# NeRdTheNed/deft4j

Measured on NVIDIA B200. Metric: input MB/s optimised (-m NONE), higher is better.
Workload: dtype u8

## Files before the change

### deft4j_b200/csrc/deft4cu.cu

```cuda
#include <algorithm>
#include <cstdio>
#include <cstdlib>
#include <cstring>
#include <memory>
#include <chrono>
#include <mutex>
#include <string>
#include <thread>
#include <vector>

#include "../../include/deft4cu.h"

namespace d4 {
static thread_local std::string g_err;
static void set_error(const std::string& s) { g_err = s; }
}

#include "write.cuh"
#include "checksum.cuh"

namespace d4 {

static int g_device = -1;
static int g_sms = 148;
// ... 255 lines not shown
    std::vector<uint32_t> chain_off;
    uint32_t parse_rewalks = 0, parse_walkers = 0;

    int parse() {
        HostTimer ht("parse");
        release_model();
        too_big = false;
        cudaEvent_t ev[4];
        for (auto& e : ev) cudaEventCreate(&e);
        descs.assign(n + 1, StreamDesc{});
        infos.assign(n, StreamInfo{});
        D4_CUDA_CHECK(dalloc(&d_gerr, 8, cs));
        D4_CUDA_CHECK(cudaMemsetAsync(d_gerr, 0, 8 * sizeof(int), cs));
        uint64_t seg_bytes = 128 << 10;
        if (const char* e = getenv("D4_SEG_BYTES")) seg_bytes = std::max<uint64_t>(64, strtoull(e, nullptr, 10));
        const uint64_t seg_bits = seg_bytes * 8;
        const uint64_t spec_max_bits = 4 * seg_bits + (1 << 20);
        wdescs.clear();
        std::vector<uint32_t> w0(n), spec_list, all_list;
        for (uint32_t i = 0; i < n; i++) {
            const uint32_t nseg = in_len[i] <= seg_bytes ? 1u : (uint32_t)((in_len[i] + seg_bytes - 1) / seg_bytes);
            w0[i] = (uint32_t)wdescs.size();
            for (uint32_t j = 0; j < nseg; j++) {
                StreamDesc d{};
                d.in_off = in_off[i]; d.in_len = in_len[i];
                d.start_bit = j == 0 ? 0 : BIT_NONE;
                d.stop_bit = nseg == 1 ? BIT_NONE : (uint64_t)(j + 1) * seg_bits;
                d.walker0 = w0[i]; d.nseg = nseg; d.spec = j == 0 ? 0 : 1;
                if (nseg == 1) { d.blk_cap = in_len[i] / 4096 + 8; d.chunk_cap = in_len[i] * 8 / CHUNK_BITS + d.blk_cap + 8; }
                else { d.blk_cap = seg_bytes / 2048 + 8; d.chunk_cap = 4 * seg_bits / CHUNK_BITS + d.blk_cap + 8; }
                if (j) spec_list.push_back((uint32_t)wdescs.size());
                all_list.push_back((uint32_t)wdescs.size());
                wdescs.push_back(d);
            }
        }
        const uint32_t W = (uint32_t)wdescs.size();
        parse_walkers = W; parse_rewalks = 0;
        std::vector<uint32_t> wstream(W);
        for (uint32_t i = 0; i < n; i++) for (uint32_t j = 0; j < wdescs[w0[i]].nseg; j++) wstream[w0[i] + j] = i;
        winfos.assign(W, StreamInfo{});
        uint32_t* d_list = nullptr;
        D4_CUDA_CHECK(dalloc(&d_descs, (size_t)W, cs));
        D4_CUDA_CHECK(dalloc(&d_infos, (size_t)W, cs));
        D4_CUDA_CHECK(dalloc(&d_list, (size_t)W, cs));
        cudaEventRecord(ev[0], cs);
        if (!spec_list.empty()) {
            D4_CUDA_CHECK(cudaMemcpyAsync(d_descs, wdescs.data(), sizeof(StreamDesc) * W, cudaMemcpyHostToDevice, cs));
            D4_CUDA_CHECK(cudaMemcpyAsync(d_list, spec_list.data(), 4 * spec_list.size(), cudaMemcpyHostToDevice, cs));
            LAUNCH(k_find, (unsigned)spec_list.size(), FIND_NT, cs, d_in, d_descs, d_list, seg_bits);
            std::vector<StreamDesc> tmp(W);
            D4_CUDA_CHECK(cudaMemcpyAsync(tmp.data(), d_descs, sizeof(StreamDesc) * W, cudaMemcpyDeviceToHost, cs));
            D4_CUDA_CHECK(cudaStreamSynchronize(cs));
            for (uint32_t w : spec_list) wdescs[w].start_bit = tmp[w].start_bit;
        }
        chain.clear(); chain_off.assign(n + 1, 0);
        std::vector<std::vector<uint32_t>> chains(n);
        std::vector<uint8_t> trunc(n, 0);
        for (int attempt = 0;; attempt++) {
            uint64_t bt = 0, ct = 0;
            for (uint32_t w = 0; w < W; w++) {
                wdescs[w].blk_base = bt; bt += wdescs[w].blk_cap;
                wdescs[w].chunk_base = ct; ct += wdescs[w].chunk_cap;
            }
            dfree(d_blocks, cs); dfree(d_chunks, cs);
            D4_CUDA_CHECK(dalloc(&d_blocks, bt, cs));
            D4_CUDA_CHECK(dalloc(&d_chunks, ct, cs));
            D4_CUDA_CHECK(cudaMemcpyAsync(d_descs, wdescs.data(), sizeof(StreamDesc) * W, cudaMemcpyHostToDevice, cs));
            D4_CUDA_CHECK(cudaMemcpyAsync(d_list, all_list.data(), 4 * (size_t)W, cudaMemcpyHostToDevice, cs));
            if (W) LAUNCH_SM(k_count, W, PARSE_NT, WIN_BYTES + WIN_SLACK + 16, cs, d_in, d_descs, d_infos, d_blocks, d_chunks, d_list, seg_bits, spec_max_bits);
            D4_CUDA_CHECK(cudaMemcpyAsync(winfos.data(), d_infos, sizeof(StreamInfo) * W, cudaMemcpyDeviceToHost, cs));
            D4_CUDA_CHECK(cudaStreamSynchronize(cs));
            if (stage && cs == own_cs) { host_release(stage); stage = nullptr; }
            std::vector<uint32_t> cur(n), pending;
            std::vector<uint8_t> fin(n, 0);
            for (uint32_t i = 0; i < n; i++) { chains[i].assign(1, w0[i]); cur[i] = w0[i]; }
            bool overflow = false;
            while (true) {
                pending.clear();
                for (uint32_t i = 0; i < n; i++) {
                    if (fin[i]) continue;
                    while (true) {
                        const StreamInfo& wi = winfos[cur[i]];
                        const StreamDesc& wd = wdescs[cur[i]];
                        if (wi.n_blocks > wd.blk_cap || wi.n_chunks > wd.chunk_cap) { overflow = true; fin[i] = 1; break; }
                        if (wi.status != ST_OK || wi.final_seen) { fin[i] = 1; break; }
                        if (wi.end_bit + 3 > in_len[i] * 8) { fin[i] = 2; break; }
                        uint64_t j = wi.end_bit / seg_bits;
                        if (j >= wd.nseg) j = wd.nseg - 1;
                        const uint32_t nx = w0[i] + (uint32_t)j;
                        if (nx <= cur[i]) {
                            set_error("parse chain did not advance");
                            return DEFT4CU_ERR_CUDA;
                        }
                        chains[i].push_back(nx);
                        cur[i] = nx;
                        if (wdescs[nx].start_bit == wi.end_bit && winfos[nx].status != ST_NONE && winfos[nx].status != ST_ABORT)
                            continue;
                        wdescs[nx].start_bit = wi.end_bit;
                        wdescs[nx].spec = 0;
                        pending.push_back(nx);
                        break;
                    }
                }
                if (pending.empty()) break;
                parse_rewalks += (uint32_t)pending.size();
                for (uint32_t w : pending)
                    D4_CUDA_CHECK(cudaMemcpyAsync(d_descs + w, &wdescs[w], sizeof(StreamDesc), cudaMemcpyHostToDevice, cs));
                D4_CUDA_CHECK(cudaMemcpyAsync(d_list, pending.data(), 4 * pending.size(), cudaMemcpyHostToDevice, cs));
                LAUNCH_SM(k_count, (unsigned)pending.size(), PARSE_NT, WIN_BYTES + WIN_SLACK + 16, cs, d_in, d_descs, d_infos, d_blocks, d_chunks, d_list, seg_bits, spec_max_bits);
                for (uint32_t w : pending)
                    D4_CUDA_CHECK(cudaMemcpyAsync(&winfos[w], d_infos + w, sizeof(StreamInfo), cudaMemcpyDeviceToHost, cs));
                D4_CUDA_CHECK(cudaStreamSynchronize(cs));
            }
            for (uint32_t i = 0; i < n; i++) trunc[i] = fin[i] == 2;
            if (!overflow) break;
            if (attempt == 3) { set_error("block/chunk capacity retry failed"); return DEFT4CU_ERR_CUDA; }
            for (uint32_t w = 0; w < W; w++) {
                if (winfos[w].status == ST_NONE) continue;
                wdescs[w].blk_cap = std::max<uint64_t>(wdescs[w].blk_cap, winfos[w].n_blocks + 8);
                wdescs[w].chunk_cap = std::max<uint64_t>(wdescs[w].chunk_cap, 2 * winfos[w].n_chunks + 8);
            }
        }
        for (uint32_t i = 0; i < n; i++) {
            StreamInfo& si = infos[i];
            si = StreamInfo{};
            si.status = ST_OK;
            for (uint32_t w : chains[i]) {
                const StreamInfo& wi = winfos[w];
                si.n_blocks += wi.n_blocks; si.n_syms += wi.n_syms; si.out_len += wi.out_len; si.n_chunks += wi.n_chunks;
                si.end_bit = wi.end_bit;
                if (wi.status != ST_OK) { si.status = wi.status >= ST_NONE ? ST_PARSE : wi.status; break; }
            }
            if (trunc[i] && si.status == ST_OK) si.status = ST_PARSE;
            if (si.out_len > 0xF0000000ull && si.status == ST_OK) si.status = ST_UNSUPPORTED;
            si.total_bits = si.end_bit;
            si.consumed = (si.end_bit + 7) >> 3;
            chain_off[i] = (uint32_t)chain.size();
            if (si.status == ST_OK) chain.insert(chain.end(), chains[i].begin(), chains[i].end());
        }
        chain_off[n] = (uint32_t)chain.size();
        dfree(d_list, cs);
        cudaEventRecord(ev[1], cs);
        uint64_t sb = 0, ob = 0;
        for (uint32_t i = 0; i < n; i++) {
            descs[i].sym_base = sb; descs[i].out_base = ob;
            for (uint32_t c = chain_off[i]; c < chain_off[i + 1]; c++) {
                StreamDesc& wd = wdescs[chain[c]];
                wd.sym_base = sb; wd.out_base = ob; wd.stream_out_base = descs[i].out_base;
                sb += winfos[chain[c]].n_syms; ob += winfos[chain[c]].out_len;
            }
        }
        descs[n].sym_base = sb; descs[n].out_base = ob;
        nsym_total = sb; nout_total = ob;
        uint64_t ob_max = 0xF8000000ull;
        if (const char* e = getenv("D4_MAX_DECODED")) ob_max = std::min<uint64_t>(ob_max, strtoull(e, nullptr, 10));
        if (ob >= ob_max) {
            too_big = true;
            for (uint32_t i = 0; i < n; i++) if (infos[i].status == ST_OK) infos[i].status = ST_UNSUPPORTED;
            set_error("decoded size of the batch exceeds 4 GiB; split the batch");
            return DEFT4CU_ERR_UNSUPPORTED;
        }
        D4_CUDA_CHECK(cudaMemcpyAsync(d_descs, wdescs.data(), sizeof(StreamDesc) * W, cudaMemcpyHostToDevice, cs));
        D4_CUDA_CHECK(dalloc(&d_sym, sb, cs));
        D4_CUDA_CHECK(dalloc(&d_symout, sb, cs));
        D4_CUDA_CHECK(dalloc(&d_out, ob + 16, cs));
        std::vector<EmitJob> jobs;
        blk_stream.clear();
// ... 316 lines not shown
    }
};

}

using namespace d4;

struct deft4cu_stream {
    std::shared_ptr<Batch> batch;
    uint32_t idx;
    bool written = false;
};
struct deft4cu_device_batch {
    std::shared_ptr<Batch> batch;
};

extern "C" {

int deft4cu_init(int device) {
    std::lock_guard<std::mutex> lk(g_mu);
    int count = 0;
    cudaError_t e = cudaGetDeviceCount(&count);
    if (e != cudaSuccess || count == 0) {
        set_error(std::string("no CUDA device: ") + cudaGetErrorString(e));
        return DEFT4CU_ERR_CUDA;
    }
    if (device < 0 || device >= count) { set_error("bad device index"); return DEFT4CU_ERR_ARG; }
    D4_CUDA_CHECK(cudaSetDevice(device));
    cudaDeviceProp p;
    D4_CUDA_CHECK(cudaGetDeviceProperties(&p, device));
    g_sms = p.multiProcessorCount;
    D4_CUDA_CHECK(cudaFuncSetAttribute(k_count, cudaFuncAttributeMaxDynamicSharedMemorySize, WIN_BYTES + WIN_SLACK + 16));
    cudaMemPool_t pool;
    if (cudaDeviceGetDefaultMemPool(&pool, device) == cudaSuccess) {
        uint64_t thr = ~0ull;
        cudaMemPoolSetAttribute(pool, cudaMemPoolAttrReleaseThreshold, &thr);
    }
    if (getenv("D4_DEBUG_LIMITS")) {
        size_t st = 0, hp = 0;
        cudaDeviceGetLimit(&st, cudaLimitStackSize);
        cudaDeviceGetLimit(&hp, cudaLimitMallocHeapSize);
        cudaFuncAttributes fa;
        cudaFuncGetAttributes(&fa, k_opt_blocks);
        fprintf(stderr, "[deft4cu] stack limit %zu heap %zu; k_opt_blocks local %zu regs %d smem %zu\n", st, hp, fa.localSizeBytes, fa.numRegs, fa.sharedSizeBytes);
        if (getenv("D4_STACK")) { cudaDeviceSetLimit(cudaLimitStackSize, atoi(getenv("D4_STACK"))); }
    }
    g_device = device;
    return DEFT4CU_OK;
}
const char* deft4cu_last_error(void) { return g_err.c_str(); }
const char* deft4cu_version(void) { return "deft4cu 0.2 (sm_100a)"; }

int deft4cu_debug_trace_begin(uint32_t cap) {
    int rc = ensure_init();
    if (rc) return rc;
    if (g_trace_dev) { cudaFree(g_trace_dev); g_trace_dev = nullptr; }
    D4_CUDA_CHECK(cudaMalloc((void**)&g_trace_dev, 16ull * cap));
    g_trace_dev_cap = cap;
    unsigned zero = 0;
    D4_CUDA_CHECK(cudaMemcpyToSymbol(g_trace, &g_trace_dev, sizeof(g_trace_dev)));
    D4_CUDA_CHECK(cudaMemcpyToSymbol(g_trace_cap, &cap, sizeof(cap)));
    D4_CUDA_CHECK(cudaMemcpyToSymbol(g_trace_n, &zero, sizeof(zero)));
    return DEFT4CU_OK;
}
int deft4cu_debug_trace_end(int64_t* dst, uint32_t cap, uint32_t* n) {
    if (!g_trace_dev) { set_error("trace not armed"); return DEFT4CU_ERR_ARG; }
    D4_CUDA_CHECK(cudaDeviceSynchronize());
    unsigned cnt = 0;
    D4_CUDA_CHECK(cudaMemcpyFromSymbol(&cnt, g_trace_n, sizeof(cnt)));
    long long* null = nullptr;
    D4_CUDA_CHECK(cudaMemcpyToSymbol(g_trace, &null, sizeof(null)));
    if (n) *n = cnt;
    uint32_t m = std::min(std::min(cnt, cap), g_trace_dev_cap);
    if (m) D4_CUDA_CHECK(cudaMemcpy(dst, g_trace_dev, 16ull * m, cudaMemcpyDeviceToHost));
    cudaFree(g_trace_dev);
    g_trace_dev = nullptr;
    return DEFT4CU_OK;
}

uint64_t deft4cu_debug_engine_launches(void) { return g_opt_launches; }

int deft4cu_debug_prof(uint64_t* dst, uint32_t n, int reset) {
#ifdef D4_PROF
    unsigned long long h[64];
    D4_CUDA_CHECK(cudaDeviceSynchronize());
    D4_CUDA_CHECK(cudaMemcpyFromSymbol(h, g_prof, sizeof(h)));
    for (uint32_t i = 0; i < n && i < 64; i++) dst[i] = h[i];
    if (reset) { memset(h, 0, sizeof h); D4_CUDA_CHECK(cudaMemcpyToSymbol(g_prof, h, sizeof(h))); }
    return DEFT4CU_OK;
#else
    (void)dst; (void)n; (void)reset;
    set_error("not a -DD4_PROF build");
    return DEFT4CU_ERR_ARG;
#endif
}

int deft4cu_stream_parse_batch(const uint8_t* const* data, const uint64_t* len, uint32_t n, deft4cu_stream** handles,
                               int32_t* status, uint64_t* consumed) {
    int rc = ensure_init();
    if (rc) return rc;
    auto b = std::make_shared<Batch>();
    rc = b->upload(data, len, n);
    if (rc) return rc;
    rc = b->parse();
    if (rc && rc != DEFT4CU_ERR_UNSUPPORTED) return rc;
    for (uint32_t i = 0; i < n; i++) {
        int st = b->infos[i].status;
        if (status) status[i] = st;
        if (consumed) consumed[i] = b->infos[i].consumed;
        handles[i] = nullptr;
        if (st == ST_OK) handles[i] = new deft4cu_stream{b, i};
    }
    return DEFT4CU_OK;
}
int deft4cu_stream_parse(const uint8_t* data, uint64_t len, deft4cu_stream** out, uint64_t* consumed) {
    int32_t st = 0;
    uint64_t c = 0;
    *out = nullptr;
    int rc = deft4cu_stream_parse_batch(&data, &len, 1, out, &st, &c);
    if (consumed) *consumed = c;
    if (rc) return rc;
    return st;
}
void deft4cu_stream_free(deft4cu_stream* s) { delete s; }

int deft4cu_stream_optimise_batch(deft4cu_stream* const* s, uint32_t n, uint32_t flags, int64_t* saved_bits) {
    std::vector<Batch*> batches;
    for (uint32_t i = 0; i < n; i++) {
        if (!s[i]) return DEFT4CU_ERR_ARG;
        if (std::find(batches.begin(), batches.end(), s[i]->batch.get()) == batches.end()) batches.push_back(s[i]->batch.get());
    }
    if (batches.size() > 1) {
        bool fresh = true;
        for (Batch* b : batches) fresh = fresh && !b->optimised && b->parsed;
        for (uint32_t i = 0; i < n && fresh; i++)
            for (uint32_t k = 0; k < i; k++) if (s[k] == s[i]) fresh = false;
        if (fresh) {
            std::vector<std::pair<Batch*, uint32_t>> src(n);
            for (uint32_t i = 0; i < n; i++) src[i] = {s[i]->batch.get(), s[i]->idx};
            auto nb = std::make_shared<Batch>();
            int rc = nb->upload_from(src);
            if (rc == DEFT4CU_OK) rc = nb->parse();
            bool same = rc == DEFT4CU_OK;
            for (uint32_t i = 0; i < n && same; i++) same = nb->infos[i].status == ST_OK;
            if (same) {
                for (uint32_t i = 0; i < n; i++) { s[i]->batch = nb; s[i]->idx = i; }
                batches.assign(1, nb.get());
            } else if (rc != DEFT4CU_OK && rc != DEFT4CU_ERR_UNSUPPORTED) return rc;
        }
    }
    int worst = DEFT4CU_OK;
    for (Batch* b : batches) {
        std::vector<uint8_t> sel(b->n, 0);
        for (uint32_t i = 0; i < n; i++) if (s[i]->batch.get() == b) sel[s[i]->idx] = 1;
        int rc = b->optimise(flags, sel);
        if (rc) worst = rc;
    }
    for (uint32_t i = 0; i < n; i++) {
        s[i]->written = false;
        if (saved_bits) saved_bits[i] = s[i]->batch->sstate[s[i]->idx].saved_bits;
    }
    return worst;
}
int deft4cu_stream_optimise(deft4cu_stream* s, uint32_t flags, int64_t* saved_bits) {
    return deft4cu_stream_optimise_batch(&s, 1, flags, saved_bits);
}
int64_t deft4cu_stream_size_bits(const deft4cu_stream* s) { return (int64_t)s->batch->sstate[s->idx].total_bits; }
uint64_t deft4cu_stream_uncompressed_len(const deft4cu_stream* s) { return s->batch->infos[s->idx].out_len; }
int deft4cu_stream_uncompressed(const deft4cu_stream* s, uint8_t* dst, uint64_t cap) {
    Batch& b = *s->batch;
    uint64_t len = b.infos[s->idx].out_len;
// ... 249 lines not shown
```

### deft4j_b200/csrc/parse.cuh

```cuda
#pragma once
#include "common.cuh"

namespace d4 {

constexpr int PARSE_NT = 1024;
constexpr int CHUNK_BITS = 256;

struct DecTab {
    uint32_t first[16];
    uint16_t count[16];
    uint16_t offs[16];
    uint16_t symtab[MAX_LL];
};

__device__ inline void build_dectab(const uint8_t* lens, int n, DecTab& t) {
    for (int l = 0; l < 16; l++) { t.count[l] = 0; t.first[l] = 0; t.offs[l] = 0; }
    for (int i = 0; i < n; i++) if (lens[i] > 0 && lens[i] < 16) t.count[lens[i]]++;
    uint32_t next = 0;
    int lastShift = 0, off = 0;
    for (int l = 1; l < 16; l++) {
        t.offs[l] = (uint16_t)off;
        off += t.count[l];
        if (t.count[l] == 0) continue;
        next <<= (l - lastShift);
        lastShift = l;
        t.first[l] = next;
        next += t.count[l];
    }
    uint16_t fill[16];
    for (int l = 0; l < 16; l++) fill[l] = t.offs[l];
    for (int i = 0; i < n; i++) if (lens[i] > 0 && lens[i] < 16) t.symtab[fill[lens[i]]++] = (uint16_t)i;
}

__device__ __forceinline__ int decode_sym(const DecTab& t, uint64_t w, int* len) {
    uint32_t code = 0;
#pragma unroll 1
    for (int l = 1; l <= 15; l++) {
        code = (code << 1) | (uint32_t)(w & 1);
        w >>= 1;
        uint32_t idx = code - t.first[l];
        if (idx < t.count[l]) { *len = l; return t.symtab[t.offs[l] + idx]; }
    }
    return -1;
}

constexpr int LUT_L_BITS = 10, LUT_D_BITS = 9;
struct DecLut {
    uint16_t lit[1 << LUT_L_BITS];
    uint16_t dst[1 << LUT_D_BITS];
};
__device__ __forceinline__ void build_lut(const DecTab& t, uint16_t* lut, int bits, int tid, int nthreads) {
    for (int i = tid; i < (1 << bits); i += nthreads) {
        uint32_t code = 0, w = (uint32_t)i;
        uint16_t e = 0;
#pragma unroll 1
        for (int l = 1; l <= bits; l++) {
            code = (code << 1) | (w & 1u);
            w >>= 1;
            const uint32_t idx = code - t.first[l];
            if (idx < t.count[l]) { e = (uint16_t)((l << 9) | t.symtab[t.offs[l] + idx]); break; }
        }
        lut[i] = e;
    }
}
__device__ __forceinline__ int decode_sym_lut(const DecTab& t, const uint16_t* lut, int bits, uint64_t w, int* len) {
    const uint32_t e = lut[(uint32_t)w & ((1u << bits) - 1u)];
    if (e) { *len = (int)(e >> 9); return (int)(e & 511u); }
    return decode_sym(t, w, len);
}

constexpr int WIN_BYTES = PARSE_NT * CHUNK_BITS / 8;
constexpr int WIN_SLACK = 64;
constexpr int HDR_STAGE = 1024;
__device__ __forceinline__ void cp_async16(void* smem, const void* gmem, int src_bytes) {
    const unsigned sa = (unsigned)__cvta_generic_to_shared(smem);
    asm volatile("cp.async.cg.shared.global [%0], [%1], 16, %2;\n" ::"r"(sa), "l"(gmem), "r"(src_bytes) : "memory");
}
__device__ __forceinline__ void cp_async_wait_all() { asm volatile("cp.async.commit_group;\ncp.async.wait_group 0;\n" ::: "memory"); }
__device__ __forceinline__ uint64_t peek_bits_smem(const uint8_t* win, uint32_t rel) {
    const uint32_t byte = rel >> 3;
    const uint64_t* q = (const uint64_t*)(win + (byte & ~7u));
    const int sh = (int)(byte & 7u) * 8;
    const uint64_t lo = q[0], hi = q[1];
    const uint64_t w = sh ? ((lo >> sh) | (hi << (64 - sh))) : lo;
    return w >> (rel & 7u);
}

struct Unit {
    int nbits;
    int outlen;
    uint32_t packed;
    int eob;
};

__device__ __forceinline__ Unit decode_unit_w(const DecTab& lit, const DecTab& dst, const DecLut& lut, uint64_t w);
__device__ __forceinline__ Unit decode_unit(const DecTab& lit, const DecTab& dst, const DecLut& lut, const uint8_t* in, uint64_t pos) {
    return decode_unit_w(lit, dst, lut, peek_bits(in, pos));
}
__device__ __forceinline__ Unit decode_unit_w(const DecTab& lit, const DecTab& dst, const DecLut& lut, uint64_t w) {
    Unit u;
    u.nbits = 0; u.outlen = 0; u.packed = 0; u.eob = 0;
    int l;
    int s = decode_sym_lut(lit, lut.lit, LUT_L_BITS, w, &l);
    if (s < 0 || s > 285) return u;
    if (s < 256) { u.nbits = l; u.outlen = 1; u.packed = (uint32_t)s; return u; }
    if (s == 256) { u.nbits = l; u.eob = 1; u.packed = 256; return u; }
    int nb = l;
    w >>= l;
    int eb = c_len_ebits[s - 257];
    int len = c_len_base[s - 257] + (int)(w & ((1u << eb) - 1));
    w >>= eb; nb += eb;
    int edge = (len == 258 && s == 284) ? 1 : 0;
    int dl;
    int ds = decode_sym_lut(dst, lut.dst, LUT_D_BITS, w, &dl);
    if (ds < 0 || ds > 29) return u;
    w >>= dl; nb += dl;
    int deb = c_dist_ebits[ds];
    int dist = c_dist_base[ds] + (int)(w & ((1u << deb) - 1));
    nb += deb;
    u.nbits = nb; u.outlen = len;
    u.packed = sym_pack_match(len, dist, edge, s);
    return u;
}

__device__ inline void fixed_lens(uint8_t* L, uint8_t* D) {
    for (int i = 0; i < 286; i++) L[i] = (i <= 143) ? 8 : (i <= 255) ? 9 : (i <= 279) ? 7 : 8;
    for (int i = 0; i < 30; i++) D[i] = 5;
}

template <class Peek>
__device__ inline uint32_t parse_dynamic_header(Peek peek, uint64_t pos, uint64_t total_bits, BlockRec& b, DecTab& scratch,
                                                uint8_t* lens) {
    uint64_t p = pos;
    if (p + 14 > total_bits) return 0;
    uint64_t w = peek(p);
    int nL = (int)(w & 31) + 257, nD = (int)((w >> 5) & 31) + 1, ncl = (int)((w >> 10) & 15) + 4;
    p += 14;
    if (p + 3ull * ncl > total_bits) return 0;
    for (int i = 0; i < 19; i++) b.hdr.CL[i] = 0;
    for (int i = 0; i < ncl; i++) {
        b.hdr.CL[c_codelen_order[i]] = (uint8_t)(peek(p) & 7);
        p += 3;
    }
    int hbits = 14 + 3 * ncl;
    build_dectab(b.hdr.CL, 19, scratch);
    int i = 0, np = 0;
    const int combined = nL + nD;
    while (i < combined) {
        if (p >= total_bits) return 0;
        w = peek(p);
        int l;
        int s = decode_sym(scratch, w, &l);
        if (s < 0) return 0;
        p += l; hbits += l; w >>= l;
        int run = 0, val;
        if (s <= 15) { lens[i++] = (uint8_t)s; val = s; }
        else if (s == 16) {
            if (i < 1) return 0;
            run = (int)(w & 3) + 3; p += 2; hbits += 2;
            if (i + run > combined) return 0;
            val = lens[i - 1];
            for (int k = 0; k < run; k++) lens[i++] = (uint8_t)val;
        } else if (s == 17) {
            run = (int)(w & 7) + 3; p += 3; hbits += 3;
            if (i + run > combined) return 0;
            val = 0;
            for (int k = 0; k < run; k++) lens[i++] = 0;
        } else {
            run = (int)(w & 127) + 11; p += 7; hbits += 7;
            if (i + run > combined) return 0;
            val = 0;
            for (int k = 0; k < run; k++) lens[i++] = 0;
        }
        if (p > total_bits) return 0;
        b.hdr.pairs[np++] = pair_pack(s, run, val);
    }
    b.hdr.np = (uint16_t)np;
    b.hdr.ncl = (uint8_t)ncl;
    b.hdr.bits = hbits;
    b.tab.nL = (uint16_t)nL; b.tab.nD = (uint16_t)nD; b.tab.type = 2;
    for (int k = 0; k < MAX_LL; k++) b.tab.L[k] = k < nL ? lens[k] : 0;
    for (int k = 0; k < MAX_D; k++) b.tab.D[k] = k < nD ? lens[nL + k] : 0;
    return (uint32_t)(p - pos);
}

constexpr int ST_OK = 0, ST_PARSE = 1, ST_UNSUPPORTED = 3, ST_NONE = 100, ST_ABORT = 101;

constexpr int FIND_NT = 256;
constexpr int FIND_TILE = FIND_NT * 8;

__device__ __forceinline__ uint64_t funnel128(uint64_t lo, uint64_t hi, int k) {
    return k ? ((lo >> k) | (hi << (64 - k))) : lo;
}

__device__ inline bool find_full_check(const uint8_t* in, uint64_t p, uint64_t total_bits) {
    uint64_t w = peek_bits(in, p);
    const int nL = (int)((w >> 3) & 31) + 257, nD = (int)((w >> 8) & 31) + 1, ncl = (int)((w >> 13) & 15) + 4;
    uint64_t q = p + 17;
    if (q + 3ull * ncl > total_bits) return false;
    uint64_t cw = peek_bits(in, q);
    uint8_t cl[19];
    for (int i = 0; i < 19; i++) cl[i] = 0;
    for (int i = 0; i < ncl; i++) cl[c_codelen_order[i]] = (uint8_t)((cw >> (3 * i)) & 7);
    q += 3ull * ncl;
    int count[8], first[8], offs[8];
    uint8_t symtab[19];
    for (int l = 0; l < 8; l++) count[l] = 0;
    for (int s = 0; s < 19; s++) count[cl[s]]++;
    count[0] = 0;
    int code = 0, off = 0;
    for (int l = 1; l < 8; l++) { code = (code + count[l - 1]) << 1; first[l] = code; offs[l] = off; off += count[l]; }
    {
        int fill[8];
        for (int l = 0; l < 8; l++) fill[l] = offs[l];
        for (int s = 0; s < 19; s++) if (cl[s]) symtab[fill[cl[s]]++] = (uint8_t)s;
    }
    const int combined = nL + nD;
    int i = 0, prev = -1, len256 = 0, nzL = 0, nzD = 0;
    uint32_t kl = 0, kd = 0;
    while (i < combined) {
        if (q >= total_bits) return false;
        w = peek_bits(in, q);
        int c = 0, l = 0, sym = -1;
        for (l = 1; l <= 7; l++) {
            c = (c << 1) | (int)(w & 1);
            w >>= 1;
            int idx = c - first[l];
            if (idx >= 0 && idx < count[l]) { sym = symtab[offs[l] + idx]; break; }
        }
        if (sym < 0) return false;
        q += l;
        int run = 1, val = sym;
        if (sym == 16) { if (prev < 0) return false; run = (int)(w & 3) + 3; q += 2; val = prev; }
        else if (sym == 17) { run = (int)(w & 7) + 3; q += 3; val = 0; }
        else if (sym == 18) { run = (int)(w & 127) + 11; q += 7; val = 0; }
        if (i + run > combined) return false;
        if (val) {
            for (int k = 0; k < run; k++) {
                const int idx = i + k;
                if (idx < nL) { kl += 32768u >> val; nzL++; if (idx == 256) len256 = val; }
                else { kd += 32768u >> val; nzD++; }
            }
            if (kl > 32768u || kd > 32768u) return false;
        }
        i += run;
        prev = val;
    }
    if (q > total_bits) return false;
    if (!len256) return false;
    if (!(kl == 32768u || (nzL == 1 && kl == 16384u))) return false;
    if (!(kd == 32768u || nzD == 0 || (nzD == 1 && kd == 16384u))) return false;
    return true;
}

__global__ void __launch_bounds__(FIND_NT)
k_find(const uint8_t* __restrict__ d_in, StreamDesc* __restrict__ descs, const uint32_t* __restrict__ list, uint64_t seg_bits) {
    const uint32_t wid = list[blockIdx.x];
    StreamDesc& sd = descs[wid];
    const uint8_t* in = d_in + sd.in_off;
    const uint64_t total_bits = sd.in_len * 8;
    const uint64_t seg_begin = (uint64_t)(wid - sd.walker0) * seg_bits;
    uint64_t seg_end = seg_begin + seg_bits;
    if (seg_end > total_bits) seg_end = total_bits;
    const int t = threadIdx.x;
    __shared__ uint16_t s_q[FIND_TILE];
    __shared__ unsigned s_n, s_best;
    uint64_t found = BIT_NONE;
    for (uint64_t tile = seg_begin; tile < seg_end && found == BIT_NONE; tile += FIND_TILE) {
        if (t == 0) { s_n = 0; s_best = 0xFFFFFFFFu; }
        __syncthreads();
        {
            const uint8_t* a = in + (tile >> 3) + t;
            const uint64_t* al = (const uint64_t*)((uintptr_t)a & ~(uintptr_t)7);
            const int sh = (int)((uintptr_t)a & 7) * 8;
            const uint64_t x0 = __ldg(al), x1 = __ldg(al + 1), x2 = __ldg(al + 2);
            const uint64_t lo = funnel128(x0, x1, sh), hi = funnel128(x1, x2, sh);
#pragma unroll
            for (int s8 = 0; s8 < 8; s8++) {
                const uint64_t p = tile + (uint64_t)t * 8 + s8;
                if (p >= seg_end || p + 17 + 12 > total_bits) continue;
                const uint64_t w1 = funnel128(lo, hi, s8);
                if (((w1 >> 1) & 3) != 2) continue;
                if (((w1 >> 3) & 31) > 29 || ((w1 >> 8) & 31) > 29) continue;
                const int ncl = (int)((w1 >> 13) & 15) + 4;
                const uint64_t cw = funnel128(lo, hi, s8 + 17);
                int kraft = 0;
                for (int i = 0; i < ncl; i++) {
                    const int v = (int)((cw >> (3 * i)) & 7);
                    kraft += v ? (128 >> v) : 0;
                }
                if (kraft != 128) continue;
                s_q[atomicAdd(&s_n, 1u)] = (uint16_t)(t * 8 + s8);
            }
        }
        __syncthreads();
        const unsigned cnt = s_n;
        for (unsigned e = (unsigned)(t & 31) * 8 + (unsigned)(t >> 5); e < cnt; e += FIND_NT) {
            const unsigned rel = s_q[e];
            if (rel < s_best && find_full_check(in, tile + rel, total_bits)) atomicMin(&s_best, rel);
        }
        __syncthreads();
        if (s_best != 0xFFFFFFFFu) found = tile + s_best;
        __syncthreads();
    }
    if (t == 0) sd.start_bit = found;
}

__global__ void __launch_bounds__(PARSE_NT, 1)
k_count(const uint8_t* __restrict__ d_in, const StreamDesc* __restrict__ descs, StreamInfo* __restrict__ infos,
        BlockRec* __restrict__ blocks, ChunkRec* __restrict__ chunks, const uint32_t* __restrict__ list,
        uint64_t seg_bits, uint64_t spec_max_bits) {
    const int sid = (int)list[blockIdx.x], t = threadIdx.x;
    const StreamDesc sd = descs[sid];
    const uint8_t* in = d_in + sd.in_off;
    const uint64_t total_bits = sd.in_len * 8;
    if (sd.start_bit == BIT_NONE) {
        if (t == 0) {
            StreamInfo si;
            si.status = ST_NONE; si.n_blocks = 0; si.n_syms = 0; si.out_len = 0; si.consumed = 0; si.n_chunks = 0;
            si.total_bits = 0; si.end_bit = BIT_NONE; si.final_seen = 0; si.pad = 0;
            infos[sid] = si;
        }
        return;
    }

    __shared__ DecTab s_lit, s_dst, s_fixlit, s_fixdst;
    __shared__ DecLut s_lut, s_fixlut;
    __shared__ BlockRec s_blk;
    __shared__ uint32_t s_start[PARSE_NT], s_end[PARSE_NT], s_cnt[PARSE_NT], s_outb[PARSE_NT];
    __shared__ uint8_t s_flag[PARSE_NT];
    __shared__ uint32_t s_scan_cnt[PARSE_NT / 32], s_scan_out[PARSE_NT / 32];
    __shared__ int s_status, s_type, s_final, s_stop;
    __shared__ uint64_t s_pos;
    extern __shared__ __align__(16) uint8_t s_win[];

    if (t == 0) {
        uint8_t L[MAX_LL], D[MAX_D];
        fixed_lens(L, D);
        L[286] = L[287] = 8;
        build_dectab(L, 288, s_fixlit);
        build_dectab(D, 30, s_fixdst);
        s_status = ST_OK;
        s_pos = sd.start_bit;
    }
    __syncthreads();
    build_lut(s_fixlit, s_fixlut.lit, LUT_L_BITS, t, PARSE_NT);
    build_lut(s_fixdst, s_fixlut.dst, LUT_D_BITS, t, PARSE_NT);
    __syncthreads();

    uint64_t n_syms = 0, out_total = 0, n_chunks = 0;
    uint32_t n_blocks = 0;
    bool done = false;

    while (!done) {
        const uint64_t hbyte = (s_pos >> 3) & ~15ull;
        {
            const int64_t valid = (int64_t)(sd.in_len + 32) - (int64_t)hbyte;
            for (int o = t * 16; o < HDR_STAGE; o += PARSE_NT * 16) {
                const int64_t left = valid - o;
                const int nb = left >= 16 ? 16 : left > 0 ? (int)left : 0;
                cp_async16(s_win + o, in + hbyte + (nb ? o : 0), nb);
            }
            cp_async_wait_all();
            __syncthreads();
        }
        if (t == 0) {
            auto peek = [&](uint64_t p) { return peek_bits_smem(s_win, (uint32_t)(p - hbyte * 8)); };
            uint64_t pos = s_pos;
            s_blk.hdr_bit = pos;
            s_blk.hdr.np = 0; s_blk.hdr.ncl = 0; s_blk.hdr.bits = 0;
            s_blk.tab.nL = 0; s_blk.tab.nD = 0;
            if (pos + 3 > total_bits) { s_status = ST_PARSE; }
            else {
                uint64_t w = peek(pos);
                s_final = (int)(w & 1);
                int type = (int)((w >> 1) & 3);
                s_type = type;
                pos += 3;
                if (type == 3) s_status = ST_PARSE;
                else if (type == 0) {
                    pos = (pos + 7) & ~7ull;
                    if (pos + 32 > total_bits) s_status = ST_PARSE;
                    else {
                        uint64_t v = peek(pos);
                        uint32_t len = (uint32_t)(v & 0xffff), nlen = (uint32_t)((v >> 16) & 0xffff);
                        pos += 32;
                        if (nlen != (~len & 0xffff)) s_status = ST_PARSE;
                        else if (pos + 8ull * len > total_bits) s_status = ST_UNSUPPORTED;
                        else {
                            s_blk.data_bit = pos;
                            s_blk.out_len = len;
                            s_blk.n_sym = 0;
                            s_blk.payload_bits = 0;
                            s_blk.tab.type = 0;
                            pos += 8ull * len;
                            s_blk.end_bit = pos;
                        }
                    }
                } else if (type == 1) {
                    s_blk.tab.type = 1;
                    s_blk.tab.nL = 286; s_blk.tab.nD = 30;
                    fixed_lens(s_blk.tab.L, s_blk.tab.D);
                    for (int k = 286; k < MAX_LL; k++) s_blk.tab.L[k] = 0;
                    for (int k = 30; k < MAX_D; k++) s_blk.tab.D[k] = 0;
                    s_blk.data_bit = pos;
                } else {
                    uint32_t used = parse_dynamic_header(peek, pos, total_bits, s_blk, s_lit, s_win + HDR_STAGE);
                    if (used == 0) s_status = ST_PARSE;
                    else {
                        pos += used;
                        s_blk.data_bit = pos;
                        build_dectab(s_blk.tab.L, s_blk.tab.nL, s_lit);
                        build_dectab(s_blk.tab.D, s_blk.tab.nD, s_dst);
                    }
                }
            }
            s_blk.type = (uint8_t)s_type;
            s_blk.bfinal = (uint8_t)s_final;
            s_pos = pos;
        }
        __syncthreads();
        if (s_status != ST_OK) break;
        const int type = s_type;
        uint32_t blk_syms = 0, blk_out = 0, blk_chunks = 0;
        const uint64_t chunk_base = n_chunks;

        if (type != 0) {
            const DecTab& lit = (type == 1) ? s_fixlit : s_lit;
            const DecTab& dst = (type == 1) ? s_fixdst : s_dst;
            if (type == 2) {
                build_lut(s_lit, s_lut.lit, LUT_L_BITS, t, PARSE_NT);
                build_lut(s_dst, s_lut.dst, LUT_D_BITS, t, PARSE_NT);
                __syncthreads();
            }
            const DecLut& lut = (type == 1) ? s_fixlut : s_lut;
            const uint64_t data_bit = s_blk.data_bit;
            uint64_t win = data_bit;
            int64_t payload = 0;
            bool eob_seen = false;
            while (!eob_seen) {
                const uint64_t wbyte = (win >> 3) & ~15ull;
                {
                    const int64_t valid = (int64_t)(sd.in_len + 32) - (int64_t)wbyte;
                    for (int o = t * 16; o < WIN_BYTES + WIN_SLACK + 16; o += PARSE_NT * 16) {
                        const int64_t left = valid - o;
                        const int nb = left >= 16 ? 16 : left > 0 ? (int)left : 0;
                        cp_async16(s_win + o, in + wbyte + (nb ? o : 0), nb);
                    }
                    cp_async_wait_all();
                    __syncthreads();
                }
                const uint32_t wrel = (uint32_t)(win - wbyte * 8);
                uint32_t start = (uint32_t)t * CHUNK_BITS;
                const uint32_t limit = (uint32_t)(t + 1) * CHUNK_BITS;
                bool need = true, changed;
                uint32_t end = 0, cnt = 0, outb = 0;
                int flag = 0;
                do {
                    if (need) {
                        uint32_t p = start;
                        cnt = 0; outb = 0; flag = 0;
                        while (p < limit) {
                            uint64_t abs = win + p;
                            if (abs >= total_bits) { flag = 2; break; }
                            Unit u = decode_unit_w(lit, dst, lut, peek_bits_smem(s_win, wrel + p));
                            if (u.nbits == 0 || abs + u.nbits > total_bits) { flag = 2; break; }
                            p += u.nbits; cnt++; outb += u.outlen;
                            if (u.eob) { flag = 1; break; }
                        }
                        end = p;
                        s_end[t] = end; s_flag[t] = (uint8_t)flag;
                    }
                    __syncthreads();
                    changed = false;
                    need = false;
                    if (t > 0 && s_flag[t - 1] == 0) {
                        uint32_t pe = s_end[t - 1];
                        if (pe != start) { start = pe; need = true; changed = true; }
                    }
                    changed = __syncthreads_or(changed);
                } while (changed);
                if (t == 0) s_stop = PARSE_NT;
                __syncthreads();
                if (flag != 0) atomicMin(&s_stop, t);
                __syncthreads();
                const int stop = s_stop;
                const bool valid = t <= stop;
                if (stop < PARSE_NT && s_flag[stop] == 2) { if (t == 0) s_status = ST_PARSE; }
                uint32_t c = valid ? cnt : 0, o = valid ? outb : 0;
                uint32_t ci = c, oi = o;
                const int lane = t & 31, wid = t >> 5;
#pragma unroll
                for (int d = 1; d < 32; d <<= 1) {
                    uint32_t a = __shfl_up_sync(0xffffffffu, ci, d), b2 = __shfl_up_sync(0xffffffffu, oi, d);
                    if (lane >= d) { ci += a; oi += b2; }
                }
                if (lane == 31) { s_scan_cnt[wid] = ci; s_scan_out[wid] = oi; }
                __syncthreads();
                if (wid == 0) {
                    uint32_t a = s_scan_cnt[lane], b2 = s_scan_out[lane];
                    uint32_t ai = a, bi = b2;
#pragma unroll
                    for (int d = 1; d < 32; d <<= 1) {
                        uint32_t x = __shfl_up_sync(0xffffffffu, ai, d), y = __shfl_up_sync(0xffffffffu, bi, d);
                        if (lane >= d) { ai += x; bi += y; }
                    }
                    s_scan_cnt[lane] = ai - a; s_scan_out[lane] = bi - b2;
                    if (lane == 31) { s_cnt[0] = ai; s_outb[0] = bi; }
                }
                __syncthreads();
                const uint32_t cbase = s_scan_cnt[wid] + ci - c, obase = s_scan_out[wid] + oi - o;
                const uint32_t wcnt = s_cnt[0], wout = s_outb[0];
                if (valid) {
                    uint64_t slot = n_chunks + (uint64_t)t;
                    if (slot < sd.chunk_cap) {
                        ChunkRec r;
                        r.start_rel = (uint32_t)(win - data_bit) + start;
                        r.sym_idx = blk_syms + cbase;
                        r.out_off = blk_out + obase;
                        r.n = cnt;
                        chunks[sd.chunk_base + slot] = r;
                    }
                }
                const int nvalid = (stop < PARSE_NT ? stop : PARSE_NT - 1) + 1;
                if (t == nvalid - 1) s_start[0] = end;
                __syncthreads();
                const uint32_t wend = s_start[0];
                payload += wend;
                win += wend;
                n_chunks += nvalid; blk_chunks += nvalid;
                blk_syms += wcnt; blk_out += wout;
                if (stop < PARSE_NT) eob_seen = true;
                if (win - data_bit > 0xFFFF0000ull || blk_syms > 0x7FFF0000u) { if (t == 0) s_status = ST_UNSUPPORTED; eob_seen = true; }
                if (sd.spec && !eob_seen && win > sd.stop_bit + spec_max_bits) { if (t == 0) s_status = ST_ABORT; eob_seen = true; }
                __syncthreads();
                if (s_status != ST_OK) break;
            }
            if (s_status != ST_OK) break;
            if (t == 0) {
                s_blk.end_bit = win;
                s_blk.n_sym = blk_syms;
                s_blk.out_len = blk_out;
                s_blk.payload_bits = payload;
                s_pos = win;
            }
        }
        if (t == 0) {
            s_blk.sym_base = n_syms;
            s_blk.out_base = out_total;
            s_blk.chunk_base = (uint32_t)chunk_base;
            s_blk.n_chunks = blk_chunks;
        }
        __syncthreads();
        if (n_blocks < sd.blk_cap) {
            const uint32_t* src = (const uint32_t*)&s_blk;
            uint32_t* dstp = (uint32_t*)&blocks[sd.blk_base + n_blocks];
            for (int k = t; k < (int)(sizeof(BlockRec) / 4); k += PARSE_NT) dstp[k] = src[k];
        }
        n_syms += (type != 0) ? s_blk.n_sym : 0;
        out_total += s_blk.out_len;
        n_blocks++;
        done = s_final != 0;
        if (!done && s_pos >= sd.stop_bit) {
            done = true;
            if (!sd.spec) {
                uint64_t j = s_pos / seg_bits;
                if (j >= sd.nseg) j = sd.nseg - 1;
                const uint64_t nxt = descs[sd.walker0 + j].start_bit;
                if (nxt != s_pos && (uint64_t)n_blocks * 2 < sd.blk_cap && n_chunks * 2 < sd.chunk_cap) done = false;
            }
        }
        if (out_total > 0xF0000000ull) { if (t == 0) s_status = ST_UNSUPPORTED; done = true; }
        __syncthreads();
    }
    if (t == 0) {
        StreamInfo si;
        si.status = s_status;
        si.n_blocks = n_blocks;
        si.n_syms = n_syms;
        si.out_len = out_total;
        si.consumed = (s_pos + 7) >> 3;
        si.n_chunks = n_chunks;
        si.total_bits = s_pos;
        si.end_bit = s_pos;
        si.final_seen = (s_status == ST_OK && s_final != 0) ? 1u : 0u;
        si.pad = 0;
        infos[sid] = si;
    }
}

struct EmitJob { uint32_t stream, block; };

__global__ void __launch_bounds__(256)
k_emit(const uint8_t* __restrict__ d_in, const StreamDesc* __restrict__ descs, const BlockRec* __restrict__ blocks,
       const ChunkRec* __restrict__ chunks, const EmitJob* __restrict__ jobs, StreamInfo* __restrict__ infos,
       uint32_t* __restrict__ sym, uint32_t* __restrict__ symout, uint8_t* __restrict__ out) {
    const EmitJob job = jobs[blockIdx.x];
    const StreamDesc sd = descs[job.stream];
    const BlockRec& b = blocks[sd.blk_base + job.block];
    const uint8_t* in = d_in + sd.in_off;
    const int t = threadIdx.x;
    if (b.type == 0) {
        const uint8_t* src = in + (b.data_bit >> 3);
        uint8_t* dst = out + sd.out_base + b.out_base;
        for (uint32_t k = t; k < b.out_len; k += blockDim.x) dst[k] = src[k];
        return;
    }
    __shared__ DecTab s_lit, s_dst;
    __shared__ DecLut s_lut;
    if (t == 0) {
        if (b.type == 1) {
            uint8_t L[MAX_LL], D[MAX_D];
            fixed_lens(L, D);
            L[286] = L[287] = 8;
            build_dectab(L, 288, s_lit);
        } else {
            build_dectab(b.tab.L, b.tab.nL, s_lit);
        }
    }
    if (t == 32) build_dectab(b.tab.D, b.tab.nD, s_dst);
    __syncthreads();
    build_lut(s_lit, s_lut.lit, LUT_L_BITS, t, (int)blockDim.x);
    build_lut(s_dst, s_lut.dst, LUT_D_BITS, t, (int)blockDim.x);
    __syncthreads();
    const uint64_t symb = sd.sym_base + b.sym_base, outb = sd.out_base + b.out_base;
    for (uint32_t c = t; c < b.n_chunks; c += blockDim.x) {
        const ChunkRec r = chunks[sd.chunk_base + b.chunk_base + c];
        uint64_t pos = b.data_bit + r.start_rel;
        uint64_t si = symb + r.sym_idx;
        uint32_t oo = (uint32_t)(outb + r.out_off);
        for (uint32_t k = 0; k < r.n; k++) {
            Unit u = decode_unit(s_lit, s_dst, s_lut, in, pos);
            pos += u.nbits;
            sym[si + k] = u.packed;
            symout[si + k] = oo;
            if (sym_is_match(u.packed) && (uint64_t)oo - sd.stream_out_base < (uint64_t)sym_dist(u.packed))
                infos[job.stream].status = ST_PARSE;
            oo += u.outlen;
        }
    }
}

__global__ void k_lz_fill(const uint32_t* __restrict__ sym, const uint32_t* __restrict__ symout, uint64_t n_sym,
                          uint8_t* __restrict__ out, uint32_t* __restrict__ ptr) {
    uint64_t i = (uint64_t)blockIdx.x * blockDim.x + threadIdx.x;
    if (i >= n_sym) return;
    uint32_t s = sym[i];
    uint32_t o = symout[i];
    if (!sym_is_match(s)) {
        if (s < 256) { out[o] = (uint8_t)s; ptr[o] = o; }
        return;
    }
    const int len = sym_len(s), dist = sym_dist(s);
    if (o < (uint32_t)dist) {
        for (int k = 0; k < len; k++) ptr[o + k] = o + k;
        return;
// ... 100 lines not shown
```

Before: 1327.

## Shrink parse CTAs, warp-parallel table builds, LUT code-length decode, early-exit fixup loop

Lowers the parse kernel block size from 1024 to 256 threads with matching launch bounds, which shrinks the per-block window and lets several CTAs share an SM. Huffman decode tables are now built by a warp using match_any instead of a single thread, and the code-length alphabet is decoded through a 7-bit LUT rather than bit-by-bit. The chunk fixup loop replaces syncthreads_or plus an atomicMin pass with warp reductions into double-buffered shared minima, and it can exit as soon as the first flagged chunk precedes the first changed chunk. Host-side chain handling now continues after a capacity overflow, and optional clock64 profiling counters are added. A smaller window means more window iterations per block and more speculation overhead for each stream.

```diff
diff --git a/deft4j_b200/csrc/deft4cu.cu b/deft4j_b200/csrc/deft4cu.cu
--- a/deft4j_b200/csrc/deft4cu.cu
+++ b/deft4j_b200/csrc/deft4cu.cu
@@ -361,7 +361,7 @@
                     while (true) {
                         const StreamInfo& wi = winfos[cur[i]];
                         const StreamDesc& wd = wdescs[cur[i]];
-                        if (wi.n_blocks > wd.blk_cap || wi.n_chunks > wd.chunk_cap) { overflow = true; fin[i] = 1; break; }
+                        if (wi.n_blocks > wd.blk_cap || wi.n_chunks > wd.chunk_cap) overflow = true;
                         if (wi.status != ST_OK || wi.final_seen) { fin[i] = 1; break; }
                         if (wi.end_bit + 3 > in_len[i] * 8) { fin[i] = 2; break; }
                         uint64_t j = wi.end_bit / seg_bits;
@@ -844,11 +844,16 @@
 
 int deft4cu_debug_prof(uint64_t* dst, uint32_t n, int reset) {
 #ifdef D4_PROF
-    unsigned long long h[64];
+    unsigned long long h[128];
     D4_CUDA_CHECK(cudaDeviceSynchronize());
-    D4_CUDA_CHECK(cudaMemcpyFromSymbol(h, g_prof, sizeof(h)));
-    for (uint32_t i = 0; i < n && i < 64; i++) dst[i] = h[i];
-    if (reset) { memset(h, 0, sizeof h); D4_CUDA_CHECK(cudaMemcpyToSymbol(g_prof, h, sizeof(h))); }
+    D4_CUDA_CHECK(cudaMemcpyFromSymbol(h, g_prof, 64 * sizeof(h[0])));
+    D4_CUDA_CHECK(cudaMemcpyFromSymbol(h + 64, g_pprof, 64 * sizeof(h[0])));
+    for (uint32_t i = 0; i < n && i < 128; i++) dst[i] = h[i];
+    if (reset) {
+        memset(h, 0, sizeof h);
+        D4_CUDA_CHECK(cudaMemcpyToSymbol(g_prof, h, 64 * sizeof(h[0])));
+        D4_CUDA_CHECK(cudaMemcpyToSymbol(g_pprof, h, 64 * sizeof(h[0])));
+    }
     return DEFT4CU_OK;
 #else
     (void)dst; (void)n; (void)reset;
diff --git a/deft4j_b200/csrc/parse.cuh b/deft4j_b200/csrc/parse.cuh
--- a/deft4j_b200/csrc/parse.cuh
+++ b/deft4j_b200/csrc/parse.cuh
@@ -3,7 +3,25 @@
 
 namespace d4 {
 
-constexpr int PARSE_NT = 1024;
+#ifdef D4_PROF
+__device__ unsigned long long g_pprof[64];
+#define PPINIT() long long pp_ = clock64()
+#define PPLAP(cat) do { if (threadIdx.x == 0) { const long long n_ = clock64(); atomicAdd(&g_pprof[cat], (unsigned long long)(n_ - pp_)); atomicAdd(&g_pprof[32 + (cat)], 1ull); pp_ = n_; } } while (0)
+#define PPCOUNT(cat, k) do { if (threadIdx.x == 0) atomicAdd(&g_pprof[32 + (cat)], (unsigned long long)(k)); } while (0)
+#else
+#define PPINIT()
+#define PPLAP(cat)
+#define PPCOUNT(cat, k)
+#endif
+enum { PP_SETUP = 0, PP_HDR_STAGE, PP_HDR_DECODE, PP_DECTAB, PP_LUT, PP_WIN_STAGE, PP_SPEC, PP_FIXUP, PP_SCAN, PP_RECORD,
+       PP_FIND_S1, PP_FIND_S2, PP_N_CHUNKS, PP_PAST_EOB, PP_FIND_SURVIVORS, PP_N_WALKERS };
+
+#ifndef D4_PARSE_NT
+#define D4_PARSE_NT 256
+#endif
+constexpr int PARSE_NT = D4_PARSE_NT;
+constexpr int PARSE_MIN_CTAS = 1024 / PARSE_NT;
+static_assert(PARSE_NT >= 64 && PARSE_NT <= 1024 && PARSE_NT % 32 == 0, "k_count needs whole warps, at least two");
 constexpr int CHUNK_BITS = 256;
 
 struct DecTab {
@@ -30,6 +48,42 @@
     uint16_t fill[16];
     for (int l = 0; l < 16; l++) fill[l] = t.offs[l];
     for (int i = 0; i < n; i++) if (lens[i] > 0 && lens[i] < 16) t.symtab[fill[lens[i]]++] = (uint16_t)i;
+}
+
+__device__ inline void build_dectab_warp(const uint8_t* lens, int n, DecTab& t, int lane) {
+    if (lane < 16) { t.count[lane] = 0; t.first[lane] = 0; t.offs[lane] = 0; }
+    __syncwarp();
+    for (int base = 0; base < n; base += 32) {
+        const int i = base + lane, l = i < n ? lens[i] : 0;
+        const unsigned grp = __match_any_sync(0xffffffffu, l);
+        if (l > 0 && l < 16 && lane == __ffs(grp) - 1) t.count[l] += (uint16_t)__popc(grp);
+        __syncwarp();
+    }
+    if (lane == 0) {
+        uint32_t next = 0;
+        int lastShift = 0, off = 0;
+        for (int l = 1; l < 16; l++) {
+            t.offs[l] = (uint16_t)off;
+            off += t.count[l];
+            if (t.count[l] == 0) continue;
+            next <<= (l - lastShift);
+            lastShift = l;
+            t.first[l] = next;
+            next += t.count[l];
+        }
+    }
+    __syncwarp();
+    for (int base = 0; base < n; base += 32) {
+        const int i = base + lane, l = i < n ? lens[i] : 0;
+        const unsigned grp = __match_any_sync(0xffffffffu, l);
+        const bool v = l > 0 && l < 16;
+        if (v) t.symtab[t.offs[l] + __popc(grp & ((1u << lane) - 1u))] = (uint16_t)i;
+        __syncwarp();
+        if (v && lane == __ffs(grp) - 1) t.offs[l] += (uint16_t)__popc(grp);
+        __syncwarp();
+    }
+    if (lane < 16) t.offs[lane] -= t.count[lane];
+    __syncwarp();
 }
 
 __device__ __forceinline__ int decode_sym(const DecTab& t, uint64_t w, int* len) {
@@ -72,6 +126,7 @@
 constexpr int WIN_BYTES = PARSE_NT * CHUNK_BITS / 8;
 constexpr int WIN_SLACK = 64;
 constexpr int HDR_STAGE = 1024;
+static_assert(HDR_STAGE + MAX_LL + MAX_D <= WIN_BYTES, "the header and its code lengths are staged in the window buffer");
 __device__ __forceinline__ void cp_async16(void* smem, const void* gmem, int src_bytes) {
     const unsigned sa = (unsigned)__cvta_generic_to_shared(smem);
     asm volatile("cp.async.cg.shared.global [%0], [%1], 16, %2;\n" ::"r"(sa), "l"(gmem), "r"(src_bytes) : "memory");
@@ -129,12 +184,11 @@
 }
 
 template <class Peek>
-__device__ inline uint32_t parse_dynamic_header(Peek peek, uint64_t pos, uint64_t total_bits, BlockRec& b, DecTab& scratch,
-                                                uint8_t* lens) {
+__device__ inline uint32_t parse_dynamic_cl(Peek peek, uint64_t pos, uint64_t total_bits, BlockRec& b) {
     uint64_t p = pos;
     if (p + 14 > total_bits) return 0;
-    uint64_t w = peek(p);
-    int nL = (int)(w & 31) + 257, nD = (int)((w >> 5) & 31) + 1, ncl = (int)((w >> 10) & 15) + 4;
+    const uint64_t w = peek(p);
+    const int nL = (int)(w & 31) + 257, nD = (int)((w >> 5) & 31) + 1, ncl = (int)((w >> 10) & 15) + 4;
     p += 14;
     if (p + 3ull * ncl > total_bits) return 0;
     for (int i = 0; i < 19; i++) b.hdr.CL[i] = 0;
@@ -142,16 +196,24 @@
         b.hdr.CL[c_codelen_order[i]] = (uint8_t)(peek(p) & 7);
         p += 3;
     }
-    int hbits = 14 + 3 * ncl;
-    build_dectab(b.hdr.CL, 19, scratch);
+    b.hdr.ncl = (uint8_t)ncl;
+    b.tab.nL = (uint16_t)nL; b.tab.nD = (uint16_t)nD;
+    return (uint32_t)(p - pos);
+}
+template <class Peek>
+__device__ inline uint32_t parse_dynamic_lens(Peek peek, uint64_t pos, uint64_t total_bits, BlockRec& b,
+                                              const uint16_t* cl_lut, uint8_t* lens) {
+    uint64_t p = pos;
+    int hbits = 14 + 3 * b.hdr.ncl;
+    const int nL = b.tab.nL, nD = b.tab.nD;
     int i = 0, np = 0;
     const int combined = nL + nD;
     while (i < combined) {
         if (p >= total_bits) return 0;
-        w = peek(p);
-        int l;
-        int s = decode_sym(scratch, w, &l);
-        if (s < 0) return 0;
+        uint64_t w = peek(p);
+        const uint32_t e = cl_lut[(uint32_t)w & 127u];
+        if (!e) return 0;
+        const int l = (int)(e >> 9), s = (int)(e & 511u);
         p += l; hbits += l; w >>= l;
         int run = 0, val;
         if (s <= 15) { lens[i++] = (uint8_t)s; val = s; }
@@ -176,9 +238,8 @@
         b.hdr.pairs[np++] = pair_pack(s, run, val);
     }
     b.hdr.np = (uint16_t)np;
-    b.hdr.ncl = (uint8_t)ncl;
     b.hdr.bits = hbits;
-    b.tab.nL = (uint16_t)nL; b.tab.nD = (uint16_t)nD; b.tab.type = 2;
+    b.tab.type = 2;
     for (int k = 0; k < MAX_LL; k++) b.tab.L[k] = k < nL ? lens[k] : 0;
     for (int k = 0; k < MAX_D; k++) b.tab.D[k] = k < nD ? lens[nL + k] : 0;
     return (uint32_t)(p - pos);
@@ -266,6 +327,7 @@
     __shared__ uint16_t s_q[FIND_TILE];
     __shared__ unsigned s_n, s_best;
     uint64_t found = BIT_NONE;
+    PPINIT();
     for (uint64_t tile = seg_begin; tile < seg_end && found == BIT_NONE; tile += FIND_TILE) {
         if (t == 0) { s_n = 0; s_best = 0xFFFFFFFFu; }
         __syncthreads();
@@ -295,18 +357,21 @@
         }
         __syncthreads();
         const unsigned cnt = s_n;
+        PPLAP(PP_FIND_S1);
+        PPCOUNT(PP_FIND_SURVIVORS, cnt);
         for (unsigned e = (unsigned)(t & 31) * 8 + (unsigned)(t >> 5); e < cnt; e += FIND_NT) {
             const unsigned rel = s_q[e];
             if (rel < s_best && find_full_check(in, tile + rel, total_bits)) atomicMin(&s_best, rel);
         }
         __syncthreads();
+        PPLAP(PP_FIND_S2);
         if (s_best != 0xFFFFFFFFu) found = tile + s_best;
         __syncthreads();
     }
     if (t == 0) sd.start_bit = found;
 }
 
-__global__ void __launch_bounds__(PARSE_NT, 1)
+__global__ void __launch_bounds__(PARSE_NT, PARSE_MIN_CTAS)
 k_count(const uint8_t* __restrict__ d_in, const StreamDesc* __restrict__ descs, StreamInfo* __restrict__ infos,
         BlockRec* __restrict__ blocks, ChunkRec* __restrict__ chunks, const uint32_t* __restrict__ list,
         uint64_t seg_bits, uint64_t spec_max_bits) {
@@ -323,30 +388,38 @@
         }
         return;
     }
+    PPINIT();
+    PPCOUNT(PP_N_WALKERS, 1);
 
     __shared__ DecTab s_lit, s_dst, s_fixlit, s_fixdst;
     __shared__ DecLut s_lut, s_fixlut;
     __shared__ BlockRec s_blk;
-    __shared__ uint32_t s_start[PARSE_NT], s_end[PARSE_NT], s_cnt[PARSE_NT], s_outb[PARSE_NT];
+    __shared__ uint32_t s_end[PARSE_NT];
     __shared__ uint8_t s_flag[PARSE_NT];
     __shared__ uint32_t s_scan_cnt[PARSE_NT / 32], s_scan_out[PARSE_NT / 32];
-    __shared__ int s_status, s_type, s_final, s_stop;
-    __shared__ uint64_t s_pos;
+    __shared__ uint32_t s_wcnt, s_wout, s_wend;
+    __shared__ int s_chg[2], s_flg[2];
+    __shared__ int s_status, s_type, s_final;
+    __shared__ uint64_t s_pos, s_clend;
     extern __shared__ __align__(16) uint8_t s_win[];
-
+    const int lane = t & 31, wid = t >> 5;
+    int par = 0;
+
+    for (int i = t; i < MAX_LL + 30; i += PARSE_NT)
+        s_win[i] = i >= MAX_LL ? 5 : (i <= 143) ? 8 : (i <= 255) ? 9 : (i <= 279) ? 7 : 8;
     if (t == 0) {
-        uint8_t L[MAX_LL], D[MAX_D];
-        fixed_lens(L, D);
-        L[286] = L[287] = 8;
-        build_dectab(L, 288, s_fixlit);
-        build_dectab(D, 30, s_fixdst);
         s_status = ST_OK;
         s_pos = sd.start_bit;
-    }
+        s_chg[0] = s_chg[1] = s_flg[0] = s_flg[1] = PARSE_NT;
+    }
+    __syncthreads();
+    if (wid == 0) build_dectab_warp(s_win, 288, s_fixlit, lane);
+    else if (wid == 1) build_dectab_warp(s_win + MAX_LL, 30, s_fixdst, lane);
     __syncthreads();
     build_lut(s_fixlit, s_fixlut.lit, LUT_L_BITS, t, PARSE_NT);
     build_lut(s_fixdst, s_fixlut.dst, LUT_D_BITS, t, PARSE_NT);
     __syncthreads();
+    PPLAP(PP_SETUP);
 
     uint64_t n_syms = 0, out_total = 0, n_chunks = 0;
     uint32_t n_blocks = 0;
@@ -364,6 +437,7 @@
             cp_async_wait_all();
             __syncthreads();
         }
+        PPLAP(PP_HDR_STAGE);
         if (t == 0) {
             auto peek = [&](uint64_t p) { return peek_bits_smem(s_win, (uint32_t)(p - hbyte * 8)); };
             uint64_t pos = s_pos;
@@ -405,14 +479,9 @@
                     for (int k = 30; k < MAX_D; k++) s_blk.tab.D[k] = 0;
                     s_blk.data_bit = pos;
                 } else {
-                    uint32_t used = parse_dynamic_header(peek, pos, total_bits, s_blk, s_lit, s_win + HDR_STAGE);
+                    const uint32_t used = parse_dynamic_cl(peek, pos, total_bits, s_blk);
                     if (used == 0) s_status = ST_PARSE;
-                    else {
-                        pos += used;
-                        s_blk.data_bit = pos;
-                        build_dectab(s_blk.tab.L, s_blk.tab.nL, s_lit);
-                        build_dectab(s_blk.tab.D, s_blk.tab.nD, s_dst);
-                    }
+                    else s_clend = pos + used;
                 }
             }
             s_blk.type = (uint8_t)s_type;
@@ -422,6 +491,27 @@
         __syncthreads();
         if (s_status != ST_OK) break;
         const int type = s_type;
+        if (type == 2) {
+            if (wid == 0) build_dectab_warp(s_blk.hdr.CL, 19, s_lit, lane);
+            __syncthreads();
+            build_lut(s_lit, s_lut.lit, 7, t, PARSE_NT);
+            __syncthreads();
+            if (t == 0) {
+                auto peek = [&](uint64_t p) { return peek_bits_smem(s_win, (uint32_t)(p - hbyte * 8)); };
+                const uint32_t used = parse_dynamic_lens(peek, s_clend, total_bits, s_blk, s_lut.lit, s_win + HDR_STAGE);
+                if (used == 0) s_status = ST_PARSE;
+                else { s_pos = s_clend + used; s_blk.data_bit = s_pos; }
+            }
+            __syncthreads();
+            PPLAP(PP_HDR_DECODE);
+            if (s_status != ST_OK) break;
+            if (wid == 0) build_dectab_warp(s_blk.tab.L, s_blk.tab.nL, s_lit, lane);
+            else if (wid == 1) build_dectab_warp(s_blk.tab.D, s_blk.tab.nD, s_dst, lane);
+            __syncthreads();
+            PPLAP(PP_DECTAB);
+        } else {
+            PPLAP(PP_HDR_DECODE);
+        }
         uint32_t blk_syms = 0, blk_out = 0, blk_chunks = 0;
         const uint64_t chunk_base = n_chunks;
 
@@ -432,6 +522,7 @@
                 build_lut(s_lit, s_lut.lit, LUT_L_BITS, t, PARSE_NT);
                 build_lut(s_dst, s_lut.dst, LUT_D_BITS, t, PARSE_NT);
                 __syncthreads();
+                PPLAP(PP_LUT);
             }
             const DecLut& lut = (type == 1) ? s_fixlut : s_lut;
             const uint64_t data_bit = s_blk.data_bit;
@@ -450,13 +541,14 @@
                     cp_async_wait_all();
                     __syncthreads();
                 }
+                PPLAP(PP_WIN_STAGE);
                 const uint32_t wrel = (uint32_t)(win - wbyte * 8);
                 uint32_t start = (uint32_t)t * CHUNK_BITS;
                 const uint32_t limit = (uint32_t)(t + 1) * CHUNK_BITS;
-                bool need = true, changed;
+                bool need = true, first = true;
                 uint32_t end = 0, cnt = 0, outb = 0;
-                int flag = 0;
-                do {
+                int flag = 0, stop;
+                while (true) {
                     if (need) {
                         uint32_t p = start;
                         cnt = 0; outb = 0; flag = 0;
@@ -472,24 +564,29 @@
                         s_end[t] = end; s_flag[t] = (uint8_t)flag;
                     }
                     __syncthreads();
-                    changed = false;
                     need = false;
                     if (t > 0 && s_flag[t - 1] == 0) {
                         uint32_t pe = s_end[t - 1];
-                        if (pe != start) { start = pe; need = true; changed = true; }
+                        if (pe != start) { start = pe; need = true; }
                     }
-                    changed = __syncthreads_or(changed);
-                } while (changed);
-                if (t == 0) s_stop = PARSE_NT;
-                __syncthreads();
-                if (flag != 0) atomicMin(&s_stop, t);
-                __syncthreads();
-                const int stop = s_stop;
+                    const int c = __reduce_min_sync(0xffffffffu, need ? t : PARSE_NT);
+                    const int f = __reduce_min_sync(0xffffffffu, flag ? t : PARSE_NT);
+                    if (lane == 0) {
+                        if (c < PARSE_NT) atomicMin(&s_chg[par], c);
+                        if (f < PARSE_NT) atomicMin(&s_flg[par], f);
+                    }
+                    if (t == 0) { s_chg[par ^ 1] = PARSE_NT; s_flg[par ^ 1] = PARSE_NT; }
+                    __syncthreads();
+                    const int fc = s_chg[par], ff = s_flg[par];
+                    par ^= 1;
+                    if (first) PPLAP(PP_SPEC); else PPLAP(PP_FIXUP);
+                    first = false;
+                    if (ff < fc || fc == PARSE_NT) { stop = ff; break; }
+                }
                 const bool valid = t <= stop;
                 if (stop < PARSE_NT && s_flag[stop] == 2) { if (t == 0) s_status = ST_PARSE; }
                 uint32_t c = valid ? cnt : 0, o = valid ? outb : 0;
                 uint32_t ci = c, oi = o;
-                const int lane = t & 31, wid = t >> 5;
 #pragma unroll
                 for (int d = 1; d < 32; d <<= 1) {
                     uint32_t a = __shfl_up_sync(0xffffffffu, ci, d), b2 = __shfl_up_sync(0xffffffffu, oi, d);
@@ -498,19 +595,20 @@
                 if (lane == 31) { s_scan_cnt[wid] = ci; s_scan_out[wid] = oi; }
                 __syncthreads();
                 if (wid == 0) {
-                    uint32_t a = s_scan_cnt[lane], b2 = s_scan_out[lane];
+                    const bool w = lane < PARSE_NT / 32;
+                    uint32_t a = w ? s_scan_cnt[lane] : 0u, b2 = w ? s_scan_out[lane] : 0u;
                     uint32_t ai = a, bi = b2;
 #pragma unroll
                     for (int d = 1; d < 32; d <<= 1) {
                         uint32_t x = __shfl_up_sync(0xffffffffu, ai, d), y = __shfl_up_sync(0xffffffffu, bi, d);
                         if (lane >= d) { ai += x; bi += y; }
                     }
-                    s_scan_cnt[lane] = ai - a; s_scan_out[lane] = bi - b2;
-                    if (lane == 31) { s_cnt[0] = ai; s_outb[0] = bi; }
+                    if (w) { s_scan_cnt[lane] = ai - a; s_scan_out[lane] = bi - b2; }
+                    if (lane == 31) { s_wcnt = ai; s_wout = bi; }
                 }
                 __syncthreads();
                 const uint32_t cbase = s_scan_cnt[wid] + ci - c, obase = s_scan_out[wid] + oi - o;
-                const uint32_t wcnt = s_cnt[0], wout = s_outb[0];
+                const uint32_t wcnt = s_wcnt, wout = s_wout;
                 if (valid) {
                     uint64_t slot = n_chunks + (uint64_t)t;
                     if (slot < sd.chunk_cap) {
@@ -523,9 +621,9 @@
                     }
                 }
                 const int nvalid = (stop < PARSE_NT ? stop : PARSE_NT - 1) + 1;
-                if (t == nvalid - 1) s_start[0] = end;
+                if (t == nvalid - 1) s_wend = end;
                 __syncthreads();
-                const uint32_t wend = s_start[0];
+                const uint32_t wend = s_wend;
                 payload += wend;
                 win += wend;
                 n_chunks += nvalid; blk_chunks += nvalid;
@@ -534,6 +632,9 @@
                 if (win - data_bit > 0xFFFF0000ull || blk_syms > 0x7FFF0000u) { if (t == 0) s_status = ST_UNSUPPORTED; eob_seen = true; }
                 if (sd.spec && !eob_seen && win > sd.stop_bit + spec_max_bits) { if (t == 0) s_status = ST_ABORT; eob_seen = true; }
                 __syncthreads();
+                PPCOUNT(PP_N_CHUNKS, nvalid);
+                PPCOUNT(PP_PAST_EOB, PARSE_NT - nvalid);
+                PPLAP(PP_SCAN);
                 if (s_status != ST_OK) break;
             }
             if (s_status != ST_OK) break;
@@ -572,6 +673,7 @@
         }
         if (out_total > 0xF0000000ull) { if (t == 0) s_status = ST_UNSUPPORTED; done = true; }
         __syncthreads();
+        PPLAP(PP_RECORD);
     }
     if (t == 0) {
         StreamInfo si;
```

New measurement: 1366, median of 6. 1.03x the previous value.
